# feiyeha/EGM-Unet

Hardware: AMD Instinct MI355X
Metric: train images/sec at 3x512x512 bs=8/GPU (higher is better)
Workload: dtype bf16; 1 GPU; EGM-UNet GRFBUNet(3,2,base_c=32) fwd+5-term-loss+bwd+SGD, 8x3x512x512 per GPU (BASELINE.json configs[1]); global_batch=8, parallelism=dp1, launch=hipGraph replay, world_size=1

## Files before the change

### egm_unet_amd/csrc/mca.hip

```cpp
#include "common.h"
#include "bn_elem.h"
#include <stdlib.h>

namespace {

inline int stream_grid(long long total_threads) {
    long long b = (total_threads + 255) / 256;
    if (b > 256 * 16) b = 256 * 16;
    if (b < 1) b = 1;
    return (int)b;
}
__device__ __forceinline__ float sigm(float v) { return 1.f / (1.f + expf(-v)); }

template <typename T, int MODE>
__global__ __launch_bounds__(256) void mca_reduce_row_kernel(const T* __restrict__ a, int lda, const T* __restrict__ b, int ldb,
                                                             float* __restrict__ sums, float* __restrict__ colp, float* __restrict__ chp,
                                                             int H, int W, int C, const float* __restrict__ scale = nullptr,
                                                             const float* __restrict__ shift = nullptr, int act = 0,
                                                             T* __restrict__ zout = nullptr, int ldz = 0) {
    __shared__ float st[2 * 256 * 8];
    __shared__ float red[16];
    const int n = blockIdx.y, h = blockIdx.x, tid = threadIdx.x, ncv = C >> 3, slots = 256 / ncv;
    const int cv = tid % ncv, slot = tid / ncv, L = H + W + C;
    const long long rowbase = ((long long)n * H + h) * W;
// ... 244 lines not shown
    const int ncv = C >> 3;
    const long long total = (long long)N * H * W * ncv;
    for (long long i = blockIdx.x * 256LL + threadIdx.x; i < total; i += (long long)gridDim.x * 256) {
        long long p; int cv; egm_divmod(i, ncv, p, cv);
        int xx, yy; egm_pix_yx(p, H, W, yy, xx);
        float c[8], s[8], v[8];
        load8(a + p * lda + cv * 8, c);
        zero8(s);
#pragma unroll
        for (int r = -1; r <= 1; ++r)
#pragma unroll
            for (int q = -1; q <= 1; ++q) {
                if (yy + r < 0 || yy + r >= H || xx + q < 0 || xx + q >= W) continue;
                load8(b + (p + (long long)r * W + q) * ldb + cv * 8, v);
#pragma unroll
                for (int j = 0; j < 8; ++j) s[j] += v[j];
            }
#pragma unroll
        for (int j = 0; j < 8; ++j) c[j] += scale * s[j] * (1.f / 9.f);
        store8(out + p * ldo + cv * 8, c);
    }
}
constexpr int MF_TY = 16, MF_TX = 16, MF_CB = 32, MF_PY = MF_TY + 4, MF_PX = MF_TX + 4, MF_UY = MF_TY + 2, MF_UX = MF_TX + 2;
template <typename T>
__global__ __launch_bounds__(256) void mca_fused_fwd_kernel(const T* __restrict__ x, int ldx, const float* __restrict__ gates,
                                                            T* __restrict__ xo, int ldxo, T* __restrict__ out, int ldo,
                                                            unsigned char* __restrict__ codes, int N, int H, int W, int C, int tiles_x,
                                                            int tiles_y, int nchunk, float inv) {
    extern __shared__ __attribute__((aligned(16))) unsigned char mf_smem[];
    T* sxo = reinterpret_cast<T*>(mf_smem);
    T* su2 = sxo + MF_PY * MF_PX * MF_CB;
    const int tid = threadIdx.x, L = H + W + C;
    int b = xcd_contiguous_item(blockIdx.x, gridDim.x);
    const int chunk = b % nchunk; b /= nchunk;
    const int tx = b % tiles_x; b /= tiles_x;
    const int ty = b % tiles_y; const int n = b / tiles_y;
    const int y0 = ty * MF_TY, x0 = tx * MF_TX, c0 = chunk * MF_CB;
    const int nvec = (C - c0 < MF_CB ? C - c0 : MF_CB) >> 3;
    const float* __restrict__ g = gates + (long long)n * L;
    const long long img = (long long)n * H * W;
    __shared__ float sgh[MF_PY], sgw[MF_PX];
    if (tid < MF_PY) { const int gy = y0 + tid - 2; sgh[tid] = (gy >= 0 && gy < H) ? g[gy] : 0.f; }
    else if (tid >= 64 && tid < 64 + MF_PX) { const int gx = x0 + tid - 64 - 2; sgw[tid - 64] = (gx >= 0 && gx < W) ? g[H + gx] : 0.f; }
    const int vt = tid & 3;
    float gc8[8], gs8[8];
#pragma unroll
    for (int j = 0; j < 8; ++j) {
        const bool okv = vt < nvec;
        gc8[j] = okv ? g[H + W + c0 + vt * 8 + j] : 0.f;
        gs8[j] = okv ? g[H + W + shuffle_src(c0 + vt * 8 + j, C)] : 0.f;
    }

    constexpr int NC = MF_TY * MF_TX * 4 / 256;
    T shv[NC][8];
#pragma unroll
    for (int k = 0; k < NC; ++k) {
        const int i = tid + k * 256, pix = i >> 2, v = i & 3, ly = pix / MF_TX, lx = pix - ly * MF_TX;
        const int gy = y0 + ly, gx = x0 + lx;
        const bool ok = v < nvec && gy < H && gx < W;
        const long long p = img + (long long)(ok ? gy : 0) * W + (ok ? gx : 0);
        const int q0 = ok ? ((c0 + v * 8) >> 2) : 0;
#pragma unroll
        for (int grp = 0; grp < 4; ++grp) {
            const T* sp = x + p * ldx + (ok ? grp * (C >> 2) : 0) + q0;
            if (sizeof(T) == 2 && ((C >> 2) & 1) == 0) {
                const uint32_t two = *reinterpret_cast<const uint32_t*>(sp);
                __builtin_memcpy(&shv[k][grp], &two, 2);
                const uint16_t hi = (uint16_t)(two >> 16);
                __builtin_memcpy(&shv[k][grp + 4], &hi, 2);
            } else {
                shv[k][grp] = sp[0]; shv[k][grp + 4] = sp[1];
            }
        }
    }
    constexpr int NA = (MF_PY * MF_PX * 4 + 255) / 256;
    uint4 raw[NA];
#pragma unroll
    for (int k = 0; k < NA; ++k) {
        const int i = tid + k * 256, pix = i >> 2, v = i & 3, py = pix / MF_PX, px = pix - py * MF_PX;
        const int gy = y0 + py - 2, gx = x0 + px - 2;
// ... 3 lines not shown
            if (sizeof(T) == 2) raw[k] = *reinterpret_cast<const uint4*>(src);
        }
    }
    __syncthreads();
#pragma unroll
    for (int k = 0; k < NA; ++k) {
        const int i = tid + k * 256, pix = i >> 2, v = i & 3, py = pix / MF_PX, px = pix - py * MF_PX;
        const int gy = y0 + py - 2, gx = x0 + px - 2;
        if (i >= MF_PY * MF_PX * 4) continue;
        float val[8];
        zero8(val);
        if (v < nvec && gy >= 0 && gy < H && gx >= 0 && gx < W) {
            const long long p = img + (long long)gy * W + gx;
            if (sizeof(T) == 2) load8(reinterpret_cast<const T*>(&raw[k]), val);
            else load8(x + p * ldx + c0 + v * 8, val);
            const float ghw = sgh[py] + sgw[px];
#pragma unroll
            for (int j = 0; j < 8; ++j) val[j] = to_f32(from_f32<T>(val[j] * ((ghw + gc8[j]) * inv)));
            if (xo != nullptr && py >= 2 && py < MF_TY + 2 && px >= 2 && px < MF_TX + 2) store8(xo + p * ldxo + c0 + v * 8, val);
        }
        store8_lds(sxo + pix * MF_CB + v * 8, val);
    }
    __syncthreads();
    for (int i = tid; i < MF_UY * MF_UX * 4; i += 256) {
        const int pix = i >> 2, v = i & 3, uy = pix / MF_UX, ux = pix - uy * MF_UX;
        const int gy = y0 + uy - 1, gx = x0 + ux - 1;
        float o2[8];
        zero8(o2);
        if (v < nvec && gy >= 0 && gy < H && gx >= 0 && gx < W) {
            float c[8], s8[8], t[8];
            zero8(s8);
            const T* ctr = sxo + ((uy + 1) * MF_PX + ux + 1) * MF_CB + v * 8;
            load8(ctr, c);
#pragma unroll
            for (int r = -1; r <= 1; ++r)
#pragma unroll
                for (int q = -1; q <= 1; ++q) {
                    load8(ctr + (r * MF_PX + q) * MF_CB, t);
#pragma unroll
                    for (int j = 0; j < 8; ++j) s8[j] += t[j];
                }
#pragma unroll
            for (int j = 0; j < 8; ++j) { const float u = c[j] - s8[j] * (1.f / 9.f); o2[j] = u * u; }
        }
        store8_lds(su2 + pix * MF_CB + v * 8, o2);
    }
    __syncthreads();
#pragma unroll
    for (int k = 0; k < NC; ++k) {
        const int i = tid + k * 256;
        const int pix = i >> 2, v = i & 3, ly = pix / MF_TX, lx = pix - ly * MF_TX;
        const int gy = y0 + ly, gx = x0 + lx;
        if (v >= nvec || gy >= H || gx >= W) continue;
        const long long p = img + (long long)gy * W + gx;
        float c[8], mx[8], mn[8], t[8], s2[8];
        int amx[8], amn[8];
        const T* ctr = sxo + ((ly + 2) * MF_PX + lx + 2) * MF_CB + v * 8;
        const T* uctr = su2 + ((ly + 1) * MF_UX + lx + 1) * MF_CB + v * 8;
        load8(ctr, c);
        zero8(s2);
#pragma unroll
        for (int j = 0; j < 8; ++j) { mx[j] = -INFINITY; mn[j] = INFINITY; amx[j] = 4; amn[j] = 4; }
#pragma unroll
        for (int r = -1; r <= 1; ++r)
#pragma unroll
            for (int q = -1; q <= 1; ++q) {
                load8(uctr + (r * MF_UX + q) * MF_CB, t);
#pragma unroll
                for (int j = 0; j < 8; ++j) s2[j] += t[j];
                if (gy + r < 0 || gy + r >= H || gx + q < 0 || gx + q >= W) continue;
// ... 68 lines not shown
                load8(du + pn * ldd + cv * 8, v);
#pragma unroll
                for (int j = 0; j < 8; ++j) sd[j] += v[j];
                load8(g + pn * ldg + cv * 8, gp);
                const uint2 cd = *reinterpret_cast<const uint2*>(codes + pn * C + cv * 8);
                const int me = (1 - r) * 3 + (1 - q);
#pragma unroll
                for (int j = 0; j < 8; ++j) {
                    const unsigned code = ((j < 4 ? cd.x : cd.y) >> ((j & 3) * 8)) & 0xffu;
                    acc[j] += gp[j] * (((int)(code & 15u) == me ? 1.f : 0.f) - ((int)(code >> 4) == me ? 1.f : 0.f));
                }
            }
        float gc[8], dc[8], o[8];
        load8(g + p * ldg + cv * 8, gc); load8(du + p * ldd + cv * 8, dc);
#pragma unroll
        for (int j = 0; j < 8; ++j) {
            const float gs = to_f32(g[p * ldg + shuffle_dst(cv * 8 + j, C)]);
            o[j] = 0.51f * gc[j] + 0.1f * gs + dc[j] - sd[j] * (1.f / 9.f) + 0.2f * acc[j];
        }
        store8(dxo + p * ldo + cv * 8, o);
    }
}
constexpr int MB_T = 16, MB_CB = 16, MB_P = MB_T + 4, MB_U = MB_T + 2;
template <typename T>
__global__ __launch_bounds__(256) void mca_bwd_fused_kernel(const unsigned char* __restrict__ codes, const T* __restrict__ xo, int ldx,
                                                            const T* __restrict__ g, int ldg, T* __restrict__ dxo, int ldo, int N, int H, int W, int C,
                                                            int tiles_x, int tiles_y, int nchunk) {
    __shared__ __attribute__((aligned(16))) T sxo[MB_P * MB_P * MB_CB];
    __shared__ __attribute__((aligned(16))) T sg[MB_P * MB_P * MB_CB];
    __shared__ __attribute__((aligned(16))) T sdu[MB_U * MB_U * MB_CB];
    __shared__ __attribute__((aligned(16))) unsigned char scd[MB_U * MB_U * MB_CB];
    const int tid = threadIdx.x;
    int b = xcd_contiguous_item(blockIdx.x, gridDim.x);
    const int chunk = b % nchunk; b /= nchunk;
    const int tx = b % tiles_x; b /= tiles_x;
    const int ty = b % tiles_y; const int n = b / tiles_y;
    const int y0 = ty * MB_T, x0 = tx * MB_T, c0 = chunk * MB_CB;
    const int nvec = (C - c0 < MB_CB ? C - c0 : MB_CB) >> 3;
    const long long img = (long long)n * H * W;
    for (int i = tid; i < MB_P * MB_P * 2; i += 256) {
        const int pix = i >> 1, v = i & 1, py = pix / MB_P, px = pix - py * MB_P;
        const int gy = y0 + py - 2, gx = x0 + px - 2;
        uint4 a = make_uint4(0, 0, 0, 0), c = make_uint4(0, 0, 0, 0);
        if (v < nvec && gy >= 0 && gy < H && gx >= 0 && gx < W) {
            const long long p = img + (long long)gy * W + gx;
            a = *reinterpret_cast<const uint4*>(xo + p * ldx + c0 + v * 8);
            c = *reinterpret_cast<const uint4*>(g + p * ldg + c0 + v * 8);
// ... 38 lines not shown
        store8_lds(sdu + pix * MB_CB + v * 8, o);
    }
    __syncthreads();
    for (int i = tid; i < MB_T * MB_T * 2; i += 256) {
        const int pix = i >> 1, v = i & 1, ly = pix / MB_T, lx = pix - ly * MB_T;
        const int gy = y0 + ly, gx = x0 + lx;
        if (v >= nvec || gy >= H || gx >= W) continue;
        const long long p = img + (long long)gy * W + gx;
        float acc[8], sd[8], t[8], gp[8];
        zero8(acc); zero8(sd);
        const T* dctr = sdu + ((ly + 1) * MB_U + lx + 1) * MB_CB + v * 8;
        const T* gctr = sg + ((ly + 2) * MB_P + lx + 2) * MB_CB + v * 8;
        const unsigned char* cctr = scd + ((ly + 1) * MB_U + lx + 1) * MB_CB + v * 8;
#pragma unroll
        for (int r = -1; r <= 1; ++r)
#pragma unroll
            for (int q = -1; q <= 1; ++q) {
                load8(dctr + (r * MB_U + q) * MB_CB, t);
#pragma unroll
                for (int j = 0; j < 8; ++j) sd[j] += t[j];
                load8(gctr + (r * MB_P + q) * MB_CB, gp);
                const uint2 cd = *reinterpret_cast<const uint2*>(cctr + (r * MB_U + q) * MB_CB);
                const int me = (1 - r) * 3 + (1 - q);
#pragma unroll
                for (int j = 0; j < 8; ++j) {
                    const unsigned code = ((j < 4 ? cd.x : cd.y) >> ((j & 3) * 8)) & 0xffu;
                    acc[j] += gp[j] * (((int)(code & 15u) == me ? 1.f : 0.f) - ((int)(code >> 4) == me ? 1.f : 0.f));
                }
            }
        float gc[8], dc[8], o[8];
        load8(gctr, gc); load8(dctr, dc);
#pragma unroll
        for (int j = 0; j < 8; ++j) {
            const float gs = to_f32(g[p * ldg + shuffle_dst(c0 + v * 8 + j, C)]);
            o[j] = 0.51f * gc[j] + 0.1f * gs + dc[j] - sd[j] * (1.f / 9.f) + 0.2f * acc[j];
        }
        store8(dxo + p * ldo + c0 + v * 8, o);
    }
}
template <typename T>
__global__ void mca_bwd_dx_kernel(const T* __restrict__ dxo, int ldd, const T* __restrict__ x, int ldx, const float* __restrict__ gates,
                                  const float* __restrict__ coef, T* __restrict__ dx, int ldo, int N, int H, int W, int C, float inv) {
    const int ncv = C >> 3, L = H + W + C;
    const long long total = (long long)N * H * W * ncv;
    for (long long i = blockIdx.x * 256LL + threadIdx.x; i < total; i += (long long)gridDim.x * 256) {
        long long p; int cv; egm_divmod(i, ncv, p, cv);
        int w, h, n; egm_pix_nyx(p, H, W, n, h, w);
        const float* g = gates + (long long)n * L;
        const float* cf = coef + (long long)n * L * 2;
        const float ghw = g[h] + g[H + w];
        const float A0 = cf[h * 2] + cf[(H + w) * 2], B0 = cf[h * 2 + 1] + cf[(H + w) * 2 + 1];
        float d[8], v[8];
        load8(dxo + p * ldd + cv * 8, d); load8(x + p * ldx + cv * 8, v);
#pragma unroll
        for (int j = 0; j < 8; ++j) {
            const int c = H + W + cv * 8 + j;
            d[j] = d[j] * (ghw + g[c]) * inv + (A0 + cf[c * 2]) + (B0 + cf[c * 2 + 1]) * v[j];
// ... 113 lines not shown
                                int W, int C, egm_stream_t s) {
    EGM_REQ_VEC("mca_stencil1", xo, ld, C); EGM_REQ_VEC("mca_stencil1", r1, ldr, C); EGM_REQ_VEC("mca_stencil1", u2, ldu, C);
    EGM_REQ_SHAPE("mca_stencil1");
    EGM_REQUIRE(C % 4 == 0 && (codes == nullptr || (reinterpret_cast<uintptr_t>(codes) & 7) == 0), "mca_stencil1: bad codes buffer");
    EGM_DISPATCH_DTYPE(dtype, hipLaunchKernelGGL((mca_stencil1_kernel<T>), dim3(EGM_MCA_GRID), dim3(256), 0, (hipStream_t)s, (const T*)xo, ld,
                                                 (T*)r1, ldr, (T*)u2, ldu, codes, N, H, W, C));
    EGM_CHECK_LAUNCH("mca_stencil1");
    return EGM_OK;
}
extern "C" int egm_add_avg3(int dtype, const void* a, int lda, const void* b, int ldb, float scale, void* out, int ldo, int N, int H, int W,
                            int C, egm_stream_t s) {
    EGM_REQ_VEC("add_avg3", a, lda, C); EGM_REQ_VEC("add_avg3", b, ldb, C); EGM_REQ_VEC("add_avg3", out, ldo, C); EGM_REQ_SHAPE("add_avg3");
    EGM_DISPATCH_DTYPE(dtype, hipLaunchKernelGGL((add_avg3_kernel<T>), dim3(EGM_MCA_GRID), dim3(256), 0, (hipStream_t)s, (const T*)a, lda,
                                                 (const T*)b, ldb, scale, (T*)out, ldo, N, H, W, C));
    EGM_CHECK_LAUNCH("add_avg3");
    return EGM_OK;
}
template <typename T>
static int launch_mca_fused(const void* x, int ldx, const float* gates, void* xo, int ldxo, void* out, int ldo, unsigned char* codes, int N, int H,
                            int W, int C, float inv, hipStream_t st) {
    const size_t smem = (size_t)(MF_PY * MF_PX + MF_UY * MF_UX) * MF_CB * sizeof(T);
    static bool attr_done = false;
    if (!attr_done) {
        hipError_t e = hipFuncSetAttribute(reinterpret_cast<const void*>(mca_fused_fwd_kernel<T>), hipFuncAttributeMaxDynamicSharedMemorySize,
                                           (int)smem);
        if (e != hipSuccess) EGM_FAIL(EGM_ERR_LAUNCH, "mca_fused_fwd: hipFuncSetAttribute: %s", hipGetErrorString(e));
        attr_done = true;
    }
    const int tiles_x = (W + MF_TX - 1) / MF_TX, tiles_y = (H + MF_TY - 1) / MF_TY, nchunk = (C + MF_CB - 1) / MF_CB;
    const long long grid = (long long)N * tiles_x * tiles_y * nchunk;
    EGM_REQUIRE(grid < (1LL << 31), "mca_fused_fwd: grid too large");
    hipLaunchKernelGGL((mca_fused_fwd_kernel<T>), dim3((unsigned)grid), dim3(256), smem, st, (const T*)x, ldx, gates, (T*)xo, ldxo, (T*)out, ldo,
                       codes, N, H, W, C, tiles_x, tiles_y, nchunk, inv);
    EGM_CHECK_LAUNCH("mca_fused_fwd");
    return EGM_OK;
}
extern "C" int egm_mca_fused_fwd(int dtype, const void* x, int ldx, const float* gates, void* xo, int ldxo, void* out, int ldo,
                                 unsigned char* codes, int N, int H, int W, int C, int no_spatial, egm_stream_t s) {
    const float inv = no_spatial ? 0.5f : 1.f / 3.f;
    EGM_REQ_VEC("mca_fused_fwd", x, ldx, C); EGM_REQ_VEC("mca_fused_fwd", out, ldo, C); EGM_REQ_SHAPE("mca_fused_fwd");
    if (xo != nullptr) EGM_REQ_VEC("mca_fused_fwd", xo, ldxo, C);
    EGM_REQUIRE(gates && C % 4 == 0 && (codes == nullptr || (reinterpret_cast<uintptr_t>(codes) & 7) == 0), "mca_fused_fwd: bad gates / codes buffer");
    if (dtype == EGM_BF16) return launch_mca_fused<bf16_t>(x, ldx, gates, xo, ldxo, out, ldo, codes, N, H, W, C, inv, (hipStream_t)s);
    if (dtype == EGM_F32) return launch_mca_fused<float>(x, ldx, gates, xo, ldxo, out, ldo, codes, N, H, W, C, inv, (hipStream_t)s);
    EGM_FAIL(EGM_ERR_ARG, "mca_fused_fwd: unknown dtype %d", dtype);
}
extern "C" int egm_mca_bwd_du(int dtype, const void* xo, int ld, const void* g, int ldg, void* du, int ldd, int N, int H, int W, int C,
                              egm_stream_t s) {
    EGM_REQ_VEC("mca_bwd_du", xo, ld, C); EGM_REQ_VEC("mca_bwd_du", g, ldg, C); EGM_REQ_VEC("mca_bwd_du", du, ldd, C); EGM_REQ_SHAPE("mca_bwd_du");
    EGM_DISPATCH_DTYPE(dtype, hipLaunchKernelGGL((mca_bwd_du_kernel<T>), dim3(EGM_MCA_GRID), dim3(256), 0, (hipStream_t)s, (const T*)xo, ld,
                                                 (const T*)g, ldg, (T*)du, ldd, N, H, W, C));
    EGM_CHECK_LAUNCH("mca_bwd_du");
    return EGM_OK;
}
extern "C" int egm_mca_bwd_dxo(int dtype, const unsigned char* codes, const void* g, int ldg, const void* du, int ldd, void* dxo, int ldo,
                               int N, int H, int W, int C, egm_stream_t s) {
    EGM_REQ_VEC("mca_bwd_dxo", g, ldg, C); EGM_REQ_VEC("mca_bwd_dxo", du, ldd, C); EGM_REQ_VEC("mca_bwd_dxo", dxo, ldo, C);
    EGM_REQ_SHAPE("mca_bwd_dxo");
    EGM_REQUIRE(codes && (reinterpret_cast<uintptr_t>(codes) & 7) == 0 && C % 4 == 0, "mca_bwd_dxo: bad codes buffer");
    EGM_DISPATCH_DTYPE(dtype, hipLaunchKernelGGL((mca_bwd_dxo_kernel<T>), dim3(EGM_MCA_GRID), dim3(256), 0, (hipStream_t)s, codes, (const T*)g,
                                                 ldg, (const T*)du, ldd, (T*)dxo, ldo, N, H, W, C));
    EGM_CHECK_LAUNCH("mca_bwd_dxo");
    return EGM_OK;
}
extern "C" int egm_mca_bwd_dudxo(int dtype, const unsigned char* codes, const void* xo, int ldxo, const void* g, int ldg, void* dxo, int ldo,
                                 int N, int H, int W, int C, egm_stream_t s) {
    EGM_REQ_VEC("mca_bwd_dudxo", xo, ldxo, C); EGM_REQ_VEC("mca_bwd_dudxo", g, ldg, C); EGM_REQ_VEC("mca_bwd_dudxo", dxo, ldo, C);
    EGM_REQ_SHAPE("mca_bwd_dudxo");
    EGM_REQUIRE(codes && (reinterpret_cast<uintptr_t>(codes) & 7) == 0 && C % 4 == 0, "mca_bwd_dudxo: bad codes buffer");
    if (dtype != EGM_BF16) EGM_FAIL(EGM_ERR_UNSUPPORTED, "mca_bwd_dudxo: bf16 only (fp32: egm_mca_bwd_du + egm_mca_bwd_dxo)");
    const int tiles_x = (W + MB_T - 1) / MB_T, tiles_y = (H + MB_T - 1) / MB_T, nchunk = (C + MB_CB - 1) / MB_CB;
    const long long grid = (long long)N * tiles_x * tiles_y * nchunk;
    EGM_REQUIRE(grid < (1LL << 31), "mca_bwd_dudxo: grid too large");
    hipLaunchKernelGGL((mca_bwd_fused_kernel<bf16_t>), dim3((unsigned)grid), dim3(256), 0, (hipStream_t)s, codes, (const bf16_t*)xo, ldxo,
                       (const bf16_t*)g, ldg, (bf16_t*)dxo, ldo, N, H, W, C, tiles_x, tiles_y, nchunk);
    EGM_CHECK_LAUNCH("mca_bwd_dudxo");
    return EGM_OK;
}
extern "C" int egm_mca_bwd_dx(int dtype, const void* dxo, int ldd, const void* x, int ldx, const float* gates, const float* coef, void* dx,
                              int ldo, int N, int H, int W, int C, int no_spatial, egm_stream_t s) {
    const float inv = no_spatial ? 0.5f : 1.f / 3.f;
    EGM_REQ_VEC("mca_bwd_dx", dxo, ldd, C); EGM_REQ_VEC("mca_bwd_dx", x, ldx, C); EGM_REQ_VEC("mca_bwd_dx", dx, ldo, C);
    EGM_REQ_SHAPE("mca_bwd_dx");
    EGM_REQUIRE(gates && coef, "mca_bwd_dx: null pointer");
    EGM_DISPATCH_DTYPE(dtype, hipLaunchKernelGGL((mca_bwd_dx_kernel<T>), dim3(EGM_MCA_GRID), dim3(256), 0, (hipStream_t)s, (const T*)dxo, ldd,
                                                 (const T*)x, ldx, gates, coef, (T*)dx, ldo, N, H, W, C, inv));
    EGM_CHECK_LAUNCH("mca_bwd_dx");
    return EGM_OK;
}
```

### egm_unet_amd/csrc/pool_up.hip

```cpp
#include "common.h"

namespace {

inline int stream_grid(long long total_threads) {
    long long b = (total_threads + 255) / 256;
    if (b > 256 * 16) b = 256 * 16;
    if (b < 1) b = 1;
    return (int)b;
}

template <typename T>
__global__ void nchw_to_nhwc_kernel(const float* __restrict__ src, T* __restrict__ dst, int ld, int N, int C, long long HW) {
    const long long total = (long long)N * HW;
    for (long long i = blockIdx.x * 256LL + threadIdx.x; i < total; i += (long long)gridDim.x * 256) {
        const long long n = i / HW, p = i - n * HW;
        for (int c0 = 0; c0 < ld; c0 += 8) {
            float v[8];
#pragma unroll
            for (int j = 0; j < 8; ++j) v[j] = (c0 + j < C) ? src[(n * C + c0 + j) * HW + p] : 0.f;
            store8(dst + i * ld + c0, v);
        }
    }
}
template <typename T>
// ... 104 lines not shown
    for (long long i = blockIdx.x * 256LL + threadIdx.x; i < total; i += (long long)gridDim.x * 256) {
        const int cv = first + (int)(i % nw); const long long p = i / nw;
        float v[8];
        if (cv < ncs) {
            load8(skip + p * lds + cv * 8, v);
        } else {
            int x, y, n; egm_pix_nyx(p, Hs, Ws, n, y, x);
            const int uy = y - py, ux = x - px, c = (cv - ncs) * 8;
            zero8(v);
            if (uy >= 0 && uy < Hu && ux >= 0 && ux < Wu) {
                const Lerp ly = lerp_coord(uy, Hl, Hu), lx = lerp_coord(ux, Wl, Wu);
                const T* b = low + (long long)n * Hl * Wl * ldl + c;
                float a[8];
                load8(b + ((long long)ly.i0 * Wl + lx.i0) * ldl, a);
#pragma unroll
                for (int j = 0; j < 8; ++j) v[j] += ly.w0 * lx.w0 * a[j];
                load8(b + ((long long)ly.i0 * Wl + lx.i1) * ldl, a);
#pragma unroll
                for (int j = 0; j < 8; ++j) v[j] += ly.w0 * lx.w1 * a[j];
                load8(b + ((long long)ly.i1 * Wl + lx.i0) * ldl, a);
#pragma unroll
                for (int j = 0; j < 8; ++j) v[j] += ly.w1 * lx.w0 * a[j];
                load8(b + ((long long)ly.i1 * Wl + lx.i1) * ldl, a);
#pragma unroll
                for (int j = 0; j < 8; ++j) v[j] += ly.w1 * lx.w1 * a[j];
            }
        }
        store8(out + p * ldo + cv * 8, v);
    }
}

template <typename T>
__global__ void upcat_bwd_low_kernel(const T* __restrict__ dout, int ldo, T* __restrict__ dlow, int ldl, int N, int Hs, int Ws,
                                     int Cs, int Hl, int Wl, int Cl) {
    const int ncl = Cl >> 3;
    const int Hu = 2 * Hl, Wu = 2 * Wl, py = (Hs - Hu) / 2, px = (Ws - Wu) / 2;
    const long long total = (long long)N * Hl * Wl * ncl;
    for (long long i = blockIdx.x * 256LL + threadIdx.x; i < total; i += (long long)gridDim.x * 256) {
        const int cv = (int)(i % ncl); long long p = i / ncl;
        int xl, yl, n; egm_pix_nyx(p, Hl, Wl, n, yl, xl);
        float acc[8]; zero8(acc);
        float wyv[6], wxv[6];
#pragma unroll
        for (int k = 0; k < 6; ++k) {
            const int uy = 2 * yl - 2 + k, ux = 2 * xl - 2 + k;
            wyv[k] = 0.f; wxv[k] = 0.f;
// ... 377 lines not shown
extern "C" int egm_maxpool2_bwd_add(int dtype, const void* x, int ldx, const void* dy, int lddy, const void* add, int ldadd, void* dx, int lddx,
                                    int N, int H, int W, int C, egm_stream_t s) {
    EGM_REQ_VEC("maxpool2_bwd_add", x, ldx, C); EGM_REQ_VEC("maxpool2_bwd_add", dy, lddy, C); EGM_REQ_VEC("maxpool2_bwd_add", add, ldadd, C);
    EGM_REQ_VEC("maxpool2_bwd_add", dx, lddx, C);
    EGM_REQUIRE(N > 0 && H >= 2 && W >= 2 && !(H & 1) && !(W & 1), "maxpool2_bwd_add: H and W must be even (got %d x %d)", H, W);
    const long long total = (long long)N * (H / 2) * (W / 2) * (C / 8);
    EGM_DISPATCH_DTYPE(dtype, hipLaunchKernelGGL((maxpool2_bwd_kernel<T>), dim3(stream_grid(total)), dim3(256), 0, (hipStream_t)s, (const T*)x, ldx,
                                                 (const T*)dy, lddy, (const T*)add, ldadd, (T*)dx, lddx, N, H, W, C));
    EGM_CHECK_LAUNCH("maxpool2_bwd_add");
    return EGM_OK;
}

extern "C" int egm_sum4_hp(int dtype, const void* a, int lda, const void* b, int ldb, const void* c, int ldc, const void* d, int ldd, void* out,
                           int ldo, int N, int H, int W, int C, egm_stream_t s) {
    EGM_REQ_VEC("sum4_hp", a, lda, C); EGM_REQ_VEC("sum4_hp", b, ldb, C); EGM_REQ_VEC("sum4_hp", out, ldo, C);
    if (c != nullptr) EGM_REQ_VEC("sum4_hp", c, ldc, C);
    if (d != nullptr) EGM_REQ_VEC("sum4_hp", d, ldd, C);
    EGM_REQUIRE(N > 0 && H > 0 && W > 0, "sum4_hp: bad shape");
    EGM_DISPATCH_DTYPE(dtype, hipLaunchKernelGGL((sum4_hp_kernel<T>), dim3(stream_grid((long long)N * H * W * (C / 8))), dim3(256), 0, (hipStream_t)s,
                                                 (const T*)a, lda, (const T*)b, ldb, (const T*)c, ldc, (const T*)d, ldd, (T*)out, ldo, N, H, W, C));
    EGM_CHECK_LAUNCH("sum4_hp");
    return EGM_OK;
}
extern "C" int egm_upcat_fwd(int dtype, const void* skip, int lds, const void* low, int ldl, void* out, int ldo, int N, int Hs, int Ws,
                             int Cs, int Hl, int Wl, int Cl, egm_stream_t s) {
    if (skip != nullptr) EGM_REQ_VEC("upcat_fwd", skip, lds, Cs);
    EGM_REQUIRE(Cs > 0 && Cs % 8 == 0, "upcat_fwd: bad Cs %d", Cs);
    EGM_REQ_VEC("upcat_fwd", low, ldl, Cl);
    EGM_REQ_VEC("upcat_fwd", out, ldo, Cs + Cl);
    EGM_REQUIRE(N > 0 && Hl > 0 && Wl > 0 && Hs >= 2 * Hl && Ws >= 2 * Wl, "upcat_fwd: skip must be at least 2x the low-res size");
    const long long total = (long long)N * Hs * Ws * ((skip ? Cs + Cl : Cl) / 8);
    EGM_DISPATCH_DTYPE(dtype, hipLaunchKernelGGL((upcat_fwd_kernel<T>), dim3(stream_grid(total)), dim3(256), 0, (hipStream_t)s,
                                                 (const T*)skip, lds, (const T*)low, ldl, (T*)out, ldo, N, Hs, Ws, Cs, Hl, Wl, Cl));
    EGM_CHECK_LAUNCH("upcat_fwd");
    return EGM_OK;
}
extern "C" int egm_upcat_bwd_low(int dtype, const void* dout, int ldo, void* dlow, int ldl, int N, int Hs, int Ws, int Cs, int Hl,
                                 int Wl, int Cl, egm_stream_t s) {
    EGM_REQ_VEC("upcat_bwd_low", dout, ldo, Cs + Cl);
    EGM_REQ_VEC("upcat_bwd_low", dlow, ldl, Cl);
    EGM_REQUIRE(N > 0 && Hl > 0 && Wl > 0 && Hs >= 2 * Hl && Ws >= 2 * Wl && Cs % 8 == 0, "upcat_bwd_low: bad shape");
    const long long total = (long long)N * Hl * Wl * (Cl / 8);
    if (dtype == EGM_BF16 && Hl >= UB_TY && Wl >= UB_TX) {
        const int tiles_y = egm_cdiv(Hl, UB_TY), tiles_x = egm_cdiv(Wl, UB_TX), nchunk = egm_cdiv(Cl, UB_CB);
        hipLaunchKernelGGL((upcat_bwd_low_tiled_kernel<bf16_t>), dim3((unsigned)((long long)N * tiles_y * tiles_x * nchunk)), dim3(256), 0, (hipStream_t)s,
                           (const bf16_t*)dout, ldo, (bf16_t*)dlow, ldl, N, Hs, Ws, Cs, Hl, Wl, Cl, tiles_x, tiles_y, nchunk);
        EGM_CHECK_LAUNCH("upcat_bwd_low");
        return EGM_OK;
    }
    EGM_DISPATCH_DTYPE(dtype, hipLaunchKernelGGL((upcat_bwd_low_kernel<T>), dim3(stream_grid(total)), dim3(256), 0, (hipStream_t)s,
                                                 (const T*)dout, ldo, (T*)dlow, ldl, N, Hs, Ws, Cs, Hl, Wl, Cl));
    EGM_CHECK_LAUNCH("upcat_bwd_low");
    return EGM_OK;
}
// ... 170 lines not shown
```

### include/egm_hip.h

```cpp
#ifndef EGM_HIP_H
#define EGM_HIP_H

#ifdef __cplusplus
extern "C" {
#endif

typedef void* egm_stream_t;

enum egm_status { EGM_OK = 0, EGM_ERR_ARG = -1, EGM_ERR_LAUNCH = -2, EGM_ERR_UNSUPPORTED = -3 };
enum egm_dtype { EGM_F32 = 0, EGM_BF16 = 1 };
enum egm_act { EGM_ACT_NONE = 0, EGM_ACT_RELU = 1, EGM_ACT_SIGMOID = 2, EGM_ACT_SILU = 3  };

int egm_version(void);
const char* egm_last_error(void);
int egm_device_ok(void);

int egm_nchw_to_nhwc(int dtype, const void* src_f32, void* dst, int ld, int N, int C, int H, int W, egm_stream_t s);
int egm_nhwc_to_nchw(int dtype, const void* src, int ld, void* dst_f32, int N, int C, int H, int W, egm_stream_t s);

int egm_conv_pack(int dtype, const void* w_oihw_f32, void* wf, void* wd, int Cout, int Cin, int KH, int KW, int groups,
                  egm_stream_t s);
int egm_conv_pack_chunk(void);
int egm_conv_pack_multi(int dtype, const void* table_dev, int n, long long total_chunks, egm_stream_t s);
int egm_group_begin(void);
// ... 138 lines not shown

int egm_maxpool2_fwd(int dtype, const void* x, int ldx, void* y, int ldy, int N, int H, int W, int C, egm_stream_t s);
int egm_maxpool2_bwd(int dtype, const void* x, int ldx, const void* dy, int lddy, void* dx, int lddx, int N, int H, int W,
                     int C, egm_stream_t s);
int egm_maxpool2_bwd_add(int dtype, const void* x, int ldx, const void* dy, int lddy, const void* add, int ldadd, void* dx, int lddx,
                         int N, int H, int W, int C, egm_stream_t s);
int egm_bn_act_fwd_pool(int dtype, const void* y, int ldy, const float* scale, const float* shift, int act, void* z, int ldz,
                        void* pooled, int ldp, int N, int H, int W, int C, egm_stream_t s);
int egm_bn_pool_bwd_blocks(int N, int H, int W, int C);
int egm_bn_pool_bwd_reduce(int dtype, const void* gskip, int ldgs, const void* gpool, int ldgp, const void* y, int ldy,
                           const float* scale, const float* shift, const float* save_mean, const float* save_rstd, int act,
                           float* partials, int N, int H, int W, int C, egm_stream_t s);
int egm_bn_pool_bwd_apply(int dtype, const void* gskip, int ldgs, const void* gpool, int ldgp, const void* y, int ldy,
                          const float* scale, const float* shift, const float* save_mean, const float* save_rstd, int act, int train,
                          const float* sums, void* dy, int lddy, int N, int H, int W, int C, egm_stream_t s);
int egm_gate3_fwd_pool(int dtype, const void* x, int ldx, const void* t, int ldt, void* out, int ldo, void* pooled, int ldp, int N,
                       int H, int W, int C, egm_stream_t s);
int egm_gate3_pool_bwd(int dtype, const void* gskip, int ldgs, const void* gpool, int ldgp, const void* x, int ldx, const void* t,
                       int ldt, void* dx, int lddx, void* dt, int lddt, int N, int H, int W, int C, egm_stream_t s);
int egm_upcat_fwd(int dtype, const void* skip, int lds, const void* low, int ldl, void* out, int ldo, int N, int Hs, int Ws,
                  int Cs, int Hl, int Wl, int Cl, egm_stream_t s);
int egm_upcat_bwd_low(int dtype, const void* dout, int ldo, void* dlow, int ldl, int N, int Hs, int Ws, int Cs, int Hl,
                      int Wl, int Cl, egm_stream_t s);

int egm_axpby(int dtype, const void* a, int lda, float alpha, const void* b, int ldb, float beta, void* out, int ldo,
              long long npix, int C, egm_stream_t s);
int egm_sum4(int dtype, const void* a, int lda, const void* b, int ldb, const void* c, int ldc, const void* d, int ldd, void* out,
             int ldo, long long npix, int C, egm_stream_t s);
int egm_sum4_hp(int dtype, const void* a, int lda, const void* b, int ldb, const void* c, int ldc, const void* d, int ldd, void* out,
                int ldo, int N, int H, int W, int C, egm_stream_t s);
int egm_vec_add_f32(float* y, const float* x, long long n, egm_stream_t s);
int egm_fill_f32(float* y, float v, long long n, egm_stream_t s);
int egm_copy_cols_f32(const float* src, int ld_src, int col0_src, float* dst, int ld_dst, int col0_dst, int rows, int ncols,
                      egm_stream_t s);

int egm_highpass3(int dtype, const void* x, int ldx, void* out, int ldo, int N, int H, int W, int C, egm_stream_t s);
int egm_gate_mul_fwd(int dtype, const void* x, int ldx, const void* w, int ldw, void* out, int ldo, long long npix, int C,
                     egm_stream_t s);
int egm_gate_mul_bwd(int dtype, const void* g, int ldg, const void* x, int ldx, const void* w, int ldw, void* dx, int lddx,
                     void* dw, int lddw, long long npix, int C, egm_stream_t s);

int egm_scale_add_relu_fwd(int dtype, const void* a, int lda, float alpha, const void* b, int ldb, void* out, int ldo,
                           long long npix, int C, egm_stream_t s);
int egm_scale_add_relu_bwd(int dtype, const void* g, int ldg, const void* out, int ldo, float alpha, void* da, int ldda,
                           void* db, int lddb, long long npix, int C, egm_stream_t s);
int egm_gate3_fwd(int dtype, const void* x, int ldx, const void* t, int ldt, void* out, int ldo, long long npix, int C,
// ... 48 lines not shown
                      float* sums, void* workspace, int N, int H, int W, int C, egm_stream_t s);
int egm_mca_gates_fwd(const float* sums, const float* w_h, const float* k_h, int ks_h, const float* w_w, const float* k_w,
                      int ks_w, const float* w_c, const float* k_c, int ks_c, float* stats, float* o, float* gates, int N, int H,
                      int W, int C, egm_stream_t s);
int egm_mca_gates_bwd(const float* dG, const float* stats, const float* o, const float* gates, const float* w_h, const float* k_h,
                      int ks_h, const float* w_w, const float* k_w, int ks_w, const float* w_c, const float* k_c, int ks_c,
                      float* dz_scratch, float* coef, float* dwts, float* dks, int N, int H, int W, int C, egm_stream_t s);
int egm_mca_xout(int dtype, const void* x, int ldx, const float* gates, void* xo, int ldo, int N, int H, int W, int C,
                 int no_spatial, egm_stream_t s);
int egm_mca_stencil1(int dtype, const void* xo, int ld, void* r1, int ldr, void* u2, int ldu, unsigned char* codes, int N, int H,
                     int W, int C, egm_stream_t s);
int egm_add_avg3(int dtype, const void* a, int lda, const void* b, int ldb, float scale, void* out, int ldo, int N, int H, int W,
                 int C, egm_stream_t s);
int egm_mca_fused_fwd(int dtype, const void* x, int ldx, const float* gates, void* xo, int ldxo, void* out, int ldo, unsigned char* codes,
                      int N, int H, int W, int C, int no_spatial, egm_stream_t s);
int egm_mca_bwd_du(int dtype, const void* xo, int ld, const void* g, int ldg, void* du, int ldd, int N, int H, int W, int C,
                   egm_stream_t s);
int egm_mca_bwd_dxo(int dtype, const unsigned char* codes, const void* g, int ldg, const void* du, int ldd, void* dxo, int ldo,
                    int N, int H, int W, int C, egm_stream_t s);
int egm_mca_bwd_dudxo(int dtype, const unsigned char* codes, const void* xo, int ldxo, const void* g, int ldg, void* dxo, int ldo,
                      int N, int H, int W, int C, egm_stream_t s);
int egm_mca_bwd_dx(int dtype, const void* dxo, int ldd, const void* x, int ldx, const float* gates, const float* coef, void* dx,
                   int ldo, int N, int H, int W, int C, int no_spatial, egm_stream_t s);

int egm_gemm(int dtype, const void* A, int lda, const void* B, int ldb, int transB, void* C, int ldc, int c_is_f32,
             const float* bias, int act, const void* R, int ldr, float alpha, int M, int N, int K, int nb1, int nb2,
             long long sA1, long long sA2, long long sB1, long long sB2, long long sC1, long long sC2, long long sR1,
             long long sR2, egm_stream_t s);
int egm_gemm_dma_mode(int mode);
int egm_attention_fused(int dtype, const void* qkv, int ld, int B, int L, int H, int head_dim, int mode, void* out, int ldo,
                        egm_stream_t s);
int egm_softmax_rows(int dtype, const float* S, int lds, void* P, int ldp, long long rows, int L, int causal, int accumulate,
                     egm_stream_t s);
int egm_layernorm(int dtype, const void* x, int ldx, const float* gamma, const float* beta, float eps, void* y, int ldy,
                  long long rows, int D, egm_stream_t s);
int egm_patchify(int dtype, const float* img_nchw, void* out, int B, int C, int H, int W, int P, egm_stream_t s);
int egm_vit_assemble(int dtype, const void* tok, const float* cls, const float* pos, void* x, int B, int Ltok, int D, egm_stream_t s);
int egm_text_embed(int dtype, const int* tokens, const float* emb, const float* pos, const float* pos_res, int split, void* x,
                   int n, int L, int D, egm_stream_t s);
int egm_film(int dtype, void* a, const void* mul, const void* add, int B, int L, int D, egm_stream_t s);
int egm_gather_rows(int dtype, const void* x, const int* idx, void* out, int n, int L, int D, egm_stream_t s);
int egm_pixel_shuffle(int dtype, const void* y, int ldy, int tok_off, int Ltot, const float* bias, float* out, int B, int g,
                      int P, egm_stream_t s);
int egm_cast_f32(int dtype, const float* src, void* dst, long long n, egm_stream_t s);

long long egm_loss_workspace(int N, int C);
// ... 150 lines not shown
```

Before: 686.4 images/s.

## Add row-sliding MCA forward, branchless bwd code decode, and tiled upcat forward

Result: no change. 685.9 images/s (-0.1%).

```diff
diff --git a/egm_unet_amd/csrc/mca.hip b/egm_unet_amd/csrc/mca.hip
--- a/egm_unet_amd/csrc/mca.hip
+++ b/egm_unet_amd/csrc/mca.hip
@@ -290,7 +290,9 @@
     }
 }
 constexpr int MF_TY = 16, MF_TX = 16, MF_CB = 32, MF_PY = MF_TY + 4, MF_PX = MF_TX + 4, MF_UY = MF_TY + 2, MF_UX = MF_TX + 2;
-template <typename T>
+constexpr int MF_BR = 6, MF_BRUNS = MF_UY / MF_BR, MF_BCP = MF_UX * 4;
+static_assert(MF_BR * MF_BRUNS == MF_UY && MF_BCP * MF_BRUNS <= 256 && MF_TX * 4 == 64, "run maps of the ROWS form");
+template <typename T, bool ROWS>
 __global__ __launch_bounds__(256) void mca_fused_fwd_kernel(const T* __restrict__ x, int ldx, const float* __restrict__ gates,
                                                             T* __restrict__ xo, int ldxo, T* __restrict__ out, int ldo,
                                                             unsigned char* __restrict__ codes, int N, int H, int W, int C, int tiles_x,
@@ -323,7 +325,7 @@
     T shv[NC][8];
 #pragma unroll
     for (int k = 0; k < NC; ++k) {
-        const int i = tid + k * 256, pix = i >> 2, v = i & 3, ly = pix / MF_TX, lx = pix - ly * MF_TX;
+        const int i = tid + k * 256, pix = i >> 2, v = i & 3, lx = pix % MF_TX, ly = ROWS ? (tid >> 6) * NC + k : pix / MF_TX;
         const int gy = y0 + ly, gx = x0 + lx;
         const bool ok = v < nvec && gy < H && gx < W;
         const long long p = img + (long long)(ok ? gy : 0) * W + (ok ? gx : 0);
@@ -373,6 +375,40 @@
         store8_lds(sxo + pix * MF_CB + v * 8, val);
     }
     __syncthreads();
+    if constexpr (ROWS) {
+        if (tid < MF_BCP * MF_BRUNS) {
+            const int run = tid / MF_BCP, cp = tid - run * MF_BCP, ux = cp >> 2, v = cp & 3, uy0 = run * MF_BR;
+            const int gx = x0 + ux - 1;
+            const bool colok = v < nvec && gx >= 0 && gx < W;
+            const T* base = sxo + (uy0 * MF_PX + ux) * MF_CB + v * 8;
+            float rw[3][3][8];
+#pragma unroll
+            for (int rr = 0; rr < 2; ++rr)
+#pragma unroll
+                for (int q = 0; q < 3; ++q) load8(base + (rr * MF_PX + q) * MF_CB, rw[rr][q]);
+#pragma unroll
+            for (int o = 0; o < MF_BR; ++o) {
+#pragma unroll
+                for (int q = 0; q < 3; ++q) load8(base + ((o + 2) * MF_PX + q) * MF_CB, rw[(o + 2) % 3][q]);
+                const int uy = uy0 + o, gy = y0 + uy - 1;
+                float o2[8];
+                zero8(o2);
+                if (colok && gy >= 0 && gy < H) {
+                    float s8[8];
+                    zero8(s8);
+#pragma unroll
+                    for (int r = 0; r < 3; ++r)
+#pragma unroll
+                        for (int q = 0; q < 3; ++q)
+#pragma unroll
+                            for (int j = 0; j < 8; ++j) s8[j] += rw[(o + r) % 3][q][j];
+#pragma unroll
+                    for (int j = 0; j < 8; ++j) { const float u = rw[(o + 1) % 3][1][j] - s8[j] * (1.f / 9.f); o2[j] = u * u; }
+                }
+                store8_lds(su2 + (uy * MF_UX + ux) * MF_CB + v * 8, o2);
+            }
+        }
+    } else
     for (int i = tid; i < MF_UY * MF_UX * 4; i += 256) {
         const int pix = i >> 2, v = i & 3, uy = pix / MF_UX, ux = pix - uy * MF_UX;
         const int gy = y0 + uy - 1, gx = x0 + ux - 1;
@@ -397,6 +433,105 @@
         store8_lds(su2 + pix * MF_CB + v * 8, o2);
     }
     __syncthreads();
+    if constexpr (ROWS) {
+        const int v = tid & 3, lx = (tid >> 2) & (MF_TX - 1), ly0 = (tid >> 6) * NC, gx = x0 + lx;
+        if (v >= nvec || gx >= W) return;
+        const bool lok = gx - 1 >= 0, rok = gx + 1 < W;
+        uint32_t o1p[NC][4], cdp[NC][2];
+        auto load4 = [](const T* p, float (&f)[4]) {
+            const uint2 a = *reinterpret_cast<const uint2*>(p);
+            f[0] = __uint_as_float(a.x << 16); f[1] = __uint_as_float(a.x & 0xffff0000u);
+            f[2] = __uint_as_float(a.y << 16); f[3] = __uint_as_float(a.y & 0xffff0000u);
+        };
+#pragma unroll
+        for (int h = 0; h < 2; ++h) {
+            float hm[3][4], hn[3][4], cc[3][4];
+            int am[3][4], an[3][4];
+            bool rowok[3];
+            const T* base = sxo + ((ly0 + 1) * MF_PX + lx + 1) * MF_CB + v * 8 + h * 4;
+#pragma unroll
+            for (int rr = 0; rr < NC + 2; ++rr) {
+                const int sl = rr % 3, gyr = y0 + ly0 - 1 + rr;
+                float t0[4], t2[4];
+                load4(base + (rr * MF_PX + 0) * MF_CB, t0);
+                load4(base + (rr * MF_PX + 1) * MF_CB, cc[sl]);
+                load4(base + (rr * MF_PX + 2) * MF_CB, t2);
+                rowok[sl] = gyr >= 0 && gyr < H;
+#pragma unroll
+                for (int j = 0; j < 4; ++j) {
+                    float m = -INFINITY, n = INFINITY;
+                    int a = 0, b = 0;
+                    if (lok && t0[j] > m) m = t0[j];
+                    if (lok && t0[j] < n) n = t0[j];
+                    if (cc[sl][j] > m) { m = cc[sl][j]; a = 1; }
+                    if (cc[sl][j] < n) { n = cc[sl][j]; b = 1; }
+                    if (rok && t2[j] > m) { m = t2[j]; a = 2; }
+                    if (rok && t2[j] < n) { n = t2[j]; b = 2; }
+                    hm[sl][j] = m; hn[sl][j] = n; am[sl][j] = a; an[sl][j] = b;
+                }
+                if (rr < 2) continue;
+                const int k = rr - 2, ly = ly0 + k;
+                if (y0 + ly >= H) continue;
+                float mx[4], mn[4];
+                int amx[4], amn[4];
+#pragma unroll
+                for (int j = 0; j < 4; ++j) { mx[j] = -INFINITY; mn[j] = INFINITY; amx[j] = 4; amn[j] = 4; }
+#pragma unroll
+                for (int r = 0; r < 3; ++r) {
+                    const int s3 = (k + r) % 3;
+                    if (!rowok[s3]) continue;
+#pragma unroll
+                    for (int j = 0; j < 4; ++j) {
+                        if (hm[s3][j] > mx[j]) { mx[j] = hm[s3][j]; amx[j] = r * 3 + am[s3][j]; }
+                        if (hn[s3][j] < mn[j]) { mn[j] = hn[s3][j]; amn[j] = r * 3 + an[s3][j]; }
+                    }
+                }
+                const float ghw = sgh[ly + 2] + sgw[lx + 2];
+                const int sc = (k + 1) % 3;
+                float o1[4];
+#pragma unroll
+                for (int j = 0; j < 4; ++j) {
+                    const float sh = to_f32(from_f32<T>(to_f32(shv[k][h * 4 + j]) * ((ghw + gs8[h * 4 + j]) * inv)));
+                    o1[j] = 0.51f * cc[sc][j] + 0.2f * (mx[j] - mn[j]) + 0.1f * sh;
+                }
+                o1p[k][h * 2] = (uint32_t)f32_to_bf16(o1[0]) | ((uint32_t)f32_to_bf16(o1[1]) << 16);
+                o1p[k][h * 2 + 1] = (uint32_t)f32_to_bf16(o1[2]) | ((uint32_t)f32_to_bf16(o1[3]) << 16);
+                cdp[k][h] = (amx[0] | (amn[0] << 4)) | ((amx[1] | (amn[1] << 4)) << 8) | ((amx[2] | (amn[2] << 4)) << 16) | ((amx[3] | (amn[3] << 4)) << 24);
+            }
+        }
+        if (codes != nullptr) {
+#pragma unroll
+            for (int k = 0; k < NC; ++k)
+                if (y0 + ly0 + k < H)
+                    *reinterpret_cast<uint2*>(codes + (img + (long long)(y0 + ly0 + k) * W + gx) * C + c0 + v * 8) = make_uint2(cdp[k][0], cdp[k][1]);
+        }
+        {
+            float rw[3][3][8];
+            const T* base = su2 + (ly0 * MF_UX + lx) * MF_CB + v * 8;
+#pragma unroll
+            for (int rr = 0; rr < NC + 2; ++rr) {
+#pragma unroll
+                for (int q = 0; q < 3; ++q) load8(base + (rr * MF_UX + q) * MF_CB, rw[rr % 3][q]);
+                if (rr < 2) continue;
+                const int k = rr - 2, gy = y0 + ly0 + k;
+                if (gy >= H) continue;
+                float s2[8], o1[8], o[8];
+                zero8(s2);
+#pragma unroll
+                for (int r = 0; r < 3; ++r)
+#pragma unroll
+                    for (int q = 0; q < 3; ++q)
+#pragma unroll
+                        for (int j = 0; j < 8; ++j) s2[j] += rw[(k + r) % 3][q][j];
+#pragma unroll
+                for (int j = 0; j < 8; ++j) o1[j] = __uint_as_float((j & 1) ? (o1p[k][j >> 1] & 0xffff0000u) : (o1p[k][j >> 1] << 16));
+#pragma unroll
+                for (int j = 0; j < 8; ++j) o[j] = o1[j] + 0.2f * s2[j] * (1.f / 9.f);
+                store8(out + (img + (long long)gy * W + gx) * ldo + c0 + v * 8, o);
+            }
+        }
+        return;
+    }
 #pragma unroll
     for (int k = 0; k < NC; ++k) {
         const int i = tid + k * 256;
@@ -511,7 +646,7 @@
     }
 }
 constexpr int MB_T = 16, MB_CB = 16, MB_P = MB_T + 4, MB_U = MB_T + 2;
-template <typename T>
+template <typename T, bool LEAN>
 __global__ __launch_bounds__(256) void mca_bwd_fused_kernel(const unsigned char* __restrict__ codes, const T* __restrict__ xo, int ldx,
                                                             const T* __restrict__ g, int ldg, T* __restrict__ dxo, int ldo, int N, int H, int W, int C,
                                                             int tiles_x, int tiles_y, int nchunk) {
@@ -596,17 +731,31 @@
                 load8(gctr + (r * MB_P + q) * MB_CB, gp);
                 const uint2 cd = *reinterpret_cast<const uint2*>(cctr + (r * MB_U + q) * MB_CB);
                 const int me = (1 - r) * 3 + (1 - q);
-#pragma unroll
-                for (int j = 0; j < 8; ++j) {
-                    const unsigned code = ((j < 4 ? cd.x : cd.y) >> ((j & 3) * 8)) & 0xffu;
-                    acc[j] += gp[j] * (((int)(code & 15u) == me ? 1.f : 0.f) - ((int)(code >> 4) == me ? 1.f : 0.f));
+                if (LEAN) {
+                    unsigned e[2];
+#pragma unroll
+                    for (int h = 0; h < 2; ++h) {
+                        const unsigned x = (h ? cd.y : cd.x) ^ ((unsigned)me * 0x11111111u);
+                        const unsigned nz = ((x & 0x77777777u) + 0x77777777u) | x;
+                        e[h] = ((nz >> 7) & 0x01010101u) + 0x01010101u - ((nz >> 3) & 0x01010101u);
+                    }
+#pragma unroll
+                    for (int j = 0; j < 8; ++j) acc[j] += gp[j] * ((float)((e[j >> 2] >> ((j & 3) * 8)) & 0xffu) - 1.f);
+                } else {
+#pragma unroll
+                    for (int j = 0; j < 8; ++j) {
+                        const unsigned code = ((j < 4 ? cd.x : cd.y) >> ((j & 3) * 8)) & 0xffu;
+                        acc[j] += gp[j] * (((int)(code & 15u) == me ? 1.f : 0.f) - ((int)(code >> 4) == me ? 1.f : 0.f));
+                    }
                 }
             }
         float gc[8], dc[8], o[8];
         load8(gctr, gc); load8(dctr, dc);
+        const int q4 = C >> 2, lq = 31 - __builtin_clz((unsigned)q4);
 #pragma unroll
         for (int j = 0; j < 8; ++j) {
-            const float gs = to_f32(g[p * ldg + shuffle_dst(c0 + v * 8 + j, C)]);
+            const int cj = c0 + v * 8 + j;
+            const float gs = to_f32(g[p * ldg + (LEAN ? ((cj & (q4 - 1)) << 2) + (cj >> lq) : shuffle_dst(cj, C))]);
             o[j] = 0.51f * gc[j] + 0.1f * gs + dc[j] - sd[j] * (1.f / 9.f) + 0.2f * acc[j];
         }
         store8(dxo + p * ldo + c0 + v * 8, o);
@@ -766,16 +915,22 @@
     const size_t smem = (size_t)(MF_PY * MF_PX + MF_UY * MF_UX) * MF_CB * sizeof(T);
     static bool attr_done = false;
     if (!attr_done) {
-        hipError_t e = hipFuncSetAttribute(reinterpret_cast<const void*>(mca_fused_fwd_kernel<T>), hipFuncAttributeMaxDynamicSharedMemorySize,
+        hipError_t e = hipFuncSetAttribute(reinterpret_cast<const void*>(mca_fused_fwd_kernel<T, false>), hipFuncAttributeMaxDynamicSharedMemorySize,
                                            (int)smem);
+        if (e == hipSuccess && sizeof(T) == 2)
+            e = hipFuncSetAttribute(reinterpret_cast<const void*>(mca_fused_fwd_kernel<bf16_t, true>), hipFuncAttributeMaxDynamicSharedMemorySize, (int)smem);
         if (e != hipSuccess) EGM_FAIL(EGM_ERR_LAUNCH, "mca_fused_fwd: hipFuncSetAttribute: %s", hipGetErrorString(e));
         attr_done = true;
     }
     const int tiles_x = (W + MF_TX - 1) / MF_TX, tiles_y = (H + MF_TY - 1) / MF_TY, nchunk = (C + MF_CB - 1) / MF_CB;
     const long long grid = (long long)N * tiles_x * tiles_y * nchunk;
     EGM_REQUIRE(grid < (1LL << 31), "mca_fused_fwd: grid too large");
-    hipLaunchKernelGGL((mca_fused_fwd_kernel<T>), dim3((unsigned)grid), dim3(256), smem, st, (const T*)x, ldx, gates, (T*)xo, ldxo, (T*)out, ldo,
-                       codes, N, H, W, C, tiles_x, tiles_y, nchunk, inv);
+    if (sizeof(T) == 2 && egm_mca_fwd_mode(-1))
+        hipLaunchKernelGGL((mca_fused_fwd_kernel<bf16_t, true>), dim3((unsigned)grid), dim3(256), smem, st, (const bf16_t*)x, ldx, gates, (bf16_t*)xo,
+                           ldxo, (bf16_t*)out, ldo, codes, N, H, W, C, tiles_x, tiles_y, nchunk, inv);
+    else
+        hipLaunchKernelGGL((mca_fused_fwd_kernel<T, false>), dim3((unsigned)grid), dim3(256), smem, st, (const T*)x, ldx, gates, (T*)xo, ldxo, (T*)out,
+                           ldo, codes, N, H, W, C, tiles_x, tiles_y, nchunk, inv);
     EGM_CHECK_LAUNCH("mca_fused_fwd");
     return EGM_OK;
 }
@@ -807,6 +962,19 @@
     EGM_CHECK_LAUNCH("mca_bwd_dxo");
     return EGM_OK;
 }
+static int g_mca_fwd_mode = -1, g_mca_bwd_mode = -1;
+extern "C" int egm_mca_fwd_mode(int mode) {
+    if (g_mca_fwd_mode < 0) g_mca_fwd_mode = getenv("EGM_MCA_FWD") ? atoi(getenv("EGM_MCA_FWD")) : 1;
+    const int old = g_mca_fwd_mode;
+    if (mode >= 0) g_mca_fwd_mode = mode;
+    return old;
+}
+extern "C" int egm_mca_bwd_mode(int mode) {
+    if (g_mca_bwd_mode < 0) g_mca_bwd_mode = getenv("EGM_MCA_BWD") ? atoi(getenv("EGM_MCA_BWD")) : 1;
+    const int old = g_mca_bwd_mode;
+    if (mode >= 0) g_mca_bwd_mode = mode;
+    return old;
+}
 extern "C" int egm_mca_bwd_dudxo(int dtype, const unsigned char* codes, const void* xo, int ldxo, const void* g, int ldg, void* dxo, int ldo,
                                  int N, int H, int W, int C, egm_stream_t s) {
     EGM_REQ_VEC("mca_bwd_dudxo", xo, ldxo, C); EGM_REQ_VEC("mca_bwd_dudxo", g, ldg, C); EGM_REQ_VEC("mca_bwd_dudxo", dxo, ldo, C);
@@ -816,8 +984,12 @@
     const int tiles_x = (W + MB_T - 1) / MB_T, tiles_y = (H + MB_T - 1) / MB_T, nchunk = (C + MB_CB - 1) / MB_CB;
     const long long grid = (long long)N * tiles_x * tiles_y * nchunk;
     EGM_REQUIRE(grid < (1LL << 31), "mca_bwd_dudxo: grid too large");
-    hipLaunchKernelGGL((mca_bwd_fused_kernel<bf16_t>), dim3((unsigned)grid), dim3(256), 0, (hipStream_t)s, codes, (const bf16_t*)xo, ldxo,
-                       (const bf16_t*)g, ldg, (bf16_t*)dxo, ldo, N, H, W, C, tiles_x, tiles_y, nchunk);
+    if (egm_mca_bwd_mode(-1) && (C & (C - 1)) == 0)
+        hipLaunchKernelGGL((mca_bwd_fused_kernel<bf16_t, true>), dim3((unsigned)grid), dim3(256), 0, (hipStream_t)s, codes, (const bf16_t*)xo, ldxo,
+                           (const bf16_t*)g, ldg, (bf16_t*)dxo, ldo, N, H, W, C, tiles_x, tiles_y, nchunk);
+    else
+        hipLaunchKernelGGL((mca_bwd_fused_kernel<bf16_t, false>), dim3((unsigned)grid), dim3(256), 0, (hipStream_t)s, codes, (const bf16_t*)xo, ldxo,
+                           (const bf16_t*)g, ldg, (bf16_t*)dxo, ldo, N, H, W, C, tiles_x, tiles_y, nchunk);
     EGM_CHECK_LAUNCH("mca_bwd_dudxo");
     return EGM_OK;
 }
diff --git a/egm_unet_amd/csrc/pool_up.hip b/egm_unet_amd/csrc/pool_up.hip
--- a/egm_unet_amd/csrc/pool_up.hip
+++ b/egm_unet_amd/csrc/pool_up.hip
@@ -1,4 +1,5 @@
 #include "common.h"
+#include <stdlib.h>
 
 namespace {
 
@@ -150,6 +151,68 @@
 #pragma unroll
                 for (int j = 0; j < 8; ++j) v[j] += ly.w1 * lx.w0 * a[j];
                 load8(b + ((long long)ly.i1 * Wl + lx.i1) * ldl, a);
+#pragma unroll
+                for (int j = 0; j < 8; ++j) v[j] += ly.w1 * lx.w1 * a[j];
+            }
+        }
+        store8(out + p * ldo + cv * 8, v);
+    }
+}
+
+constexpr int UF_TY = 8, UF_TX = 32, UF_NV = 4;
+static_assert(UF_TY * UF_TX == 256, "one pixel of the tile per thread and pass");
+template <typename T>
+__global__ __launch_bounds__(256) void upcat_fwd_tiled_kernel(const T* __restrict__ skip, int lds, const T* __restrict__ low, int ldl, T* __restrict__ out,
+                                                              int ldo, int N, int Hs, int Ws, int Cs, int Hl, int Wl, int Cl, int tiles_x, int tiles_y,
+                                                              int nchunk) {
+    __shared__ Lerp sly[UF_TY], slx[UF_TX];
+    const int ncs = Cs >> 3, ncv = (Cs + Cl) >> 3, first = skip ? 0 : ncs;
+    const int Hu = 2 * Hl, Wu = 2 * Wl, py = (Hs - Hu) / 2, px = (Ws - Wu) / 2;
+    const int tid = threadIdx.x;
+    int b = xcd_contiguous_item(blockIdx.x, gridDim.x);
+    const int chunk = b % nchunk; b /= nchunk;
+    const int tx = b % tiles_x; b /= tiles_x;
+    const int ty = b % tiles_y; const int n = b / tiles_y;
+    const int y0 = ty * UF_TY, x0 = tx * UF_TX;
+    if (tid < UF_TY) {
+        const int uy = y0 + tid - py;
+        Lerp l; l.i0 = -1; l.i1 = -1; l.w0 = 0.f; l.w1 = 0.f;
+        if (uy >= 0 && uy < Hu) l = lerp_coord(uy, Hl, Hu);
+        sly[tid] = l;
+    } else if (tid >= 64 && tid < 64 + UF_TX) {
+        const int ux = x0 + tid - 64 - px;
+        Lerp l; l.i0 = -1; l.i1 = -1; l.w0 = 0.f; l.w1 = 0.f;
+        if (ux >= 0 && ux < Wu) l = lerp_coord(ux, Wl, Wu);
+        slx[tid - 64] = l;
+    }
+    __syncthreads();
+    const T* lowb = low + (long long)n * Hl * Wl * ldl;
+#pragma unroll
+    for (int k = 0; k < UF_NV; ++k) {
+        const int e = tid + k * 256, cv = first + chunk * UF_NV + (e & (UF_NV - 1)), pix = e / UF_NV, r = pix / UF_TX, q = pix % UF_TX;
+        const int y = y0 + r, x = x0 + q;
+        if (cv >= ncv || y >= Hs || x >= Ws) continue;
+        const long long p = ((long long)n * Hs + y) * Ws + x;
+        float v[8];
+        if (cv < ncs) {
+            load8(skip + p * lds + cv * 8, v);
+        } else {
+            const Lerp ly = sly[r], lx = slx[q];
+            const int c = (cv - ncs) * 8;
+            zero8(v);
+            if (ly.i0 >= 0 && lx.i0 >= 0) {
+                const T* b0 = lowb + c;
+                float a[8];
+                load8(b0 + ((long long)ly.i0 * Wl + lx.i0) * ldl, a);
+#pragma unroll
+                for (int j = 0; j < 8; ++j) v[j] += ly.w0 * lx.w0 * a[j];
+                load8(b0 + ((long long)ly.i0 * Wl + lx.i1) * ldl, a);
+#pragma unroll
+                for (int j = 0; j < 8; ++j) v[j] += ly.w0 * lx.w1 * a[j];
+                load8(b0 + ((long long)ly.i1 * Wl + lx.i0) * ldl, a);
+#pragma unroll
+                for (int j = 0; j < 8; ++j) v[j] += ly.w1 * lx.w0 * a[j];
+                load8(b0 + ((long long)ly.i1 * Wl + lx.i1) * ldl, a);
 #pragma unroll
                 for (int j = 0; j < 8; ++j) v[j] += ly.w1 * lx.w1 * a[j];
             }
@@ -573,6 +636,13 @@
     EGM_CHECK_LAUNCH("sum4_hp");
     return EGM_OK;
 }
+static int g_upcat_mode = -1;
+extern "C" int egm_upcat_mode(int mode) {
+    if (g_upcat_mode < 0) g_upcat_mode = getenv("EGM_UPCAT") ? atoi(getenv("EGM_UPCAT")) : 1;
+    const int old = g_upcat_mode;
+    if (mode >= 0) g_upcat_mode = mode;
+    return old;
+}
 extern "C" int egm_upcat_fwd(int dtype, const void* skip, int lds, const void* low, int ldl, void* out, int ldo, int N, int Hs, int Ws,
                              int Cs, int Hl, int Wl, int Cl, egm_stream_t s) {
     if (skip != nullptr) EGM_REQ_VEC("upcat_fwd", skip, lds, Cs);
@@ -581,6 +651,17 @@
     EGM_REQ_VEC("upcat_fwd", out, ldo, Cs + Cl);
     EGM_REQUIRE(N > 0 && Hl > 0 && Wl > 0 && Hs >= 2 * Hl && Ws >= 2 * Wl, "upcat_fwd: skip must be at least 2x the low-res size");
     const long long total = (long long)N * Hs * Ws * ((skip ? Cs + Cl : Cl) / 8);
+    if (dtype == EGM_BF16 && egm_upcat_mode(-1)) {
+        const int tiles_x = (Ws + UF_TX - 1) / UF_TX, tiles_y = (Hs + UF_TY - 1) / UF_TY;
+        const int nchunk = (((Cs + Cl) >> 3) - (skip ? 0 : Cs >> 3) + UF_NV - 1) / UF_NV;
+        const long long grid = (long long)N * tiles_y * tiles_x * nchunk;
+        if (grid < (1LL << 31)) {
+            hipLaunchKernelGGL((upcat_fwd_tiled_kernel<bf16_t>), dim3((unsigned)grid), dim3(256), 0, (hipStream_t)s, (const bf16_t*)skip, lds,
+                               (const bf16_t*)low, ldl, (bf16_t*)out, ldo, N, Hs, Ws, Cs, Hl, Wl, Cl, tiles_x, tiles_y, nchunk);
+            EGM_CHECK_LAUNCH("upcat_fwd");
+            return EGM_OK;
+        }
+    }
     EGM_DISPATCH_DTYPE(dtype, hipLaunchKernelGGL((upcat_fwd_kernel<T>), dim3(stream_grid(total)), dim3(256), 0, (hipStream_t)s,
                                                  (const T*)skip, lds, (const T*)low, ldl, (T*)out, ldo, N, Hs, Ws, Cs, Hl, Wl, Cl));
     EGM_CHECK_LAUNCH("upcat_fwd");
diff --git a/include/egm_hip.h b/include/egm_hip.h
--- a/include/egm_hip.h
+++ b/include/egm_hip.h
@@ -184,6 +184,7 @@
                   int Cs, int Hl, int Wl, int Cl, egm_stream_t s);
 int egm_upcat_bwd_low(int dtype, const void* dout, int ldo, void* dlow, int ldl, int N, int Hs, int Ws, int Cs, int Hl,
                       int Wl, int Cl, egm_stream_t s);
+int egm_upcat_mode(int mode);
 
 int egm_axpby(int dtype, const void* a, int lda, float alpha, const void* b, int ldb, float beta, void* out, int ldo,
               long long npix, int C, egm_stream_t s);
@@ -278,6 +279,8 @@
                       int N, int H, int W, int C, egm_stream_t s);
 int egm_mca_bwd_dx(int dtype, const void* dxo, int ldd, const void* x, int ldx, const float* gates, const float* coef, void* dx,
                    int ldo, int N, int H, int W, int C, int no_spatial, egm_stream_t s);
+int egm_mca_fwd_mode(int mode);
+int egm_mca_bwd_mode(int mode);
 
 int egm_gemm(int dtype, const void* A, int lda, const void* B, int ldb, int transB, void* C, int ldc, int c_is_f32,
              const float* bias, int act, const void* R, int ldr, float alpha, int M, int N, int K, int nb1, int nb2,
```
